# learningOrchestra/learningOrchestra

Measured on NVIDIA H100. Metric: rows/sec project+cast+histogram 100M×32 fp64→fp32; HBM GB/s vs peak @1/2/4/8 GPU, higher is better.
Workload: dtype f64->f32

## Files before the change

include/loexec.h:

```cpp
#ifndef LOEXEC_H
#define LOEXEC_H

#include <stddef.h>
#include <stdint.h>

#ifdef __cplusplus
extern "C" {
#endif

#define LO_ABI_VERSION 3

#define LO_OK                    0
#define LO_ERR_INVALID          -1
#define LO_ERR_CUDA             -2
#define LO_ERR_NOMEM            -3
#define LO_ERR_NOT_IMPLEMENTED  -4
#define LO_ERR_NO_DEVICE        -5
#define LO_ERR_ALIGNMENT        -6

#define LO_F64 1
#define LO_F32 2
#define LO_U8  3
#define LO_U32 4

// ... 43 lines not shown
                  void *base_dev, int64_t pitch_bytes, lo_table **out);
int lo_table_free(lo_ctx *ctx, lo_table *t);
int lo_table_info(const lo_table *t, int *dtype, int64_t *nrows, int32_t *ncols,
                  int64_t *pitch_bytes, void **base_dev);
int lo_table_upload_col(lo_ctx *ctx, lo_table *t, int32_t col, int64_t row0,
                        const void *host, int64_t nrows);
int lo_table_download_col(lo_ctx *ctx, const lo_table *t, int32_t col, int64_t row0,
                          void *host, int64_t nrows, void *stream);
int lo_table_fill_synthetic_dev(lo_ctx *ctx, lo_table *t, int kind, uint64_t seed,
                                int64_t row_offset, double lo, double hi, void *stream);
int lo_table_checksum(lo_ctx *ctx, const lo_table *t, int32_t col, int64_t row_offset,
                      uint64_t *out);

int lo_selftest_fastdiv(lo_ctx *ctx, float lo, float hi, int32_t nbins, int *fast_path_used,
                        uint64_t *mismatches);

int lo_project_cast_dev(lo_ctx *ctx, const lo_table *in, const int32_t *col_idx, int32_t k,
                        lo_table *out, void *stream);
int lo_project_cast_hist_dev(lo_ctx *ctx, const lo_table *in, const int32_t *col_idx, int32_t k,
                             lo_table *out, const lo_hist_spec *spec, uint64_t *counts_dev,
                             void *stream);
int lo_hist_u8_cols_dev(lo_ctx *ctx, const lo_table *in, const int32_t *col_idx, int32_t k,
                        uint64_t *counts_dev, void *stream);
int lo_minmax_cast_dev(lo_ctx *ctx, const lo_table *in, const int32_t *col_idx, int32_t k,
                       uint64_t *out_dev, void *stream);
int lo_minmax_decode(const uint64_t *raw, int32_t k, float *mins, float *maxs, uint64_t *nfinite);
int lo_counts_alloc(lo_ctx *ctx, int64_t n, uint64_t **out_dev);
int lo_counts_free(lo_ctx *ctx, uint64_t *counts_dev);
int lo_counts_zero_dev(lo_ctx *ctx, uint64_t *counts_dev, int64_t n, void *stream);
int lo_counts_download(lo_ctx *ctx, const uint64_t *counts_dev, int64_t n, uint64_t *host,
// ... 75 lines not shown
```

learningorchestra_b200/_native.py:

```python
from __future__ import annotations

import ctypes as C
from pathlib import Path

import os

LIB_PATH = Path(os.environ.get("LOEXEC_LIB") or Path(__file__).resolve().parent / "lib" / "libloexec.so")

LO_OK = 0
LO_ERR_INVALID = -1
LO_ERR_CUDA = -2
LO_ERR_NOMEM = -3
LO_ERR_NOT_IMPLEMENTED = -4
LO_ERR_NO_DEVICE = -5
LO_ERR_ALIGNMENT = -6

LO_F64, LO_F32, LO_U8, LO_U32 = 1, 2, 3, 4
LO_SYNTH_UNIFORM, LO_SYNTH_EDGES, LO_SYNTH_CONSTCOL, LO_SYNTH_MNIST_U8 = 0, 1, 2, 3
LO_MAX_BINS = 65536
LO_MERGE_AUTO, LO_MERGE_PEER, LO_MERGE_NCCL = 0, 1, 2
LO_GROUP_BCAST = 1
LO_GROUP_INDEPENDENT = 2
LO_GROUP_BLOB_BYTES = 512
LO_GROUP_MAX_DEVICES = 16
# ... 39 lines not shown
    "lo_set_tma": (C.c_int, [_P, C.c_int]),
    "lo_launch_count": (C.c_int, [_P, C.POINTER(C.c_int64)]),
    "lo_host_alloc": (C.c_int, [_P, C.c_size_t, C.POINTER(_P)]),
    "lo_host_alloc_flags": (C.c_int, [_P, C.c_size_t, C.c_int32, C.POINTER(_P)]),
    "lo_host_free": (C.c_int, [_P, _P]),
    "lo_table_alloc": (C.c_int, [_P, C.c_int, C.c_int64, C.c_int32, C.POINTER(_P)]),
    "lo_table_wrap": (C.c_int, [_P, C.c_int, C.c_int64, C.c_int32, _P, C.c_int64, C.POINTER(_P)]),
    "lo_table_free": (C.c_int, [_P, _P]),
    "lo_table_info": (C.c_int, [_P, C.POINTER(C.c_int), C.POINTER(C.c_int64), C.POINTER(C.c_int32),
                                C.POINTER(C.c_int64), C.POINTER(_P)]),
    "lo_table_upload_col": (C.c_int, [_P, _P, C.c_int32, C.c_int64, _P, C.c_int64]),
    "lo_table_download_col": (C.c_int, [_P, _P, C.c_int32, C.c_int64, _P, C.c_int64, _P]),
    "lo_table_fill_synthetic_dev": (C.c_int, [_P, _P, C.c_int, C.c_uint64, C.c_int64, C.c_double, C.c_double, _P]),
    "lo_table_checksum": (C.c_int, [_P, _P, C.c_int32, C.c_int64, C.POINTER(C.c_uint64)]),
    "lo_selftest_fastdiv": (C.c_int, [_P, C.c_float, C.c_float, C.c_int32, C.POINTER(C.c_int), C.POINTER(C.c_uint64)]),
    "lo_minmax_cast_dev": (C.c_int, [_P, _P, C.POINTER(C.c_int32), C.c_int32, _P, _P]),
    "lo_minmax_decode": (C.c_int, [_P, C.c_int32, _P, _P, _P]),
    "lo_project_cast_dev": (C.c_int, [_P, _P, C.POINTER(C.c_int32), C.c_int32, _P, _P]),
    "lo_project_cast_hist_dev": (C.c_int, [_P, _P, C.POINTER(C.c_int32), C.c_int32, _P, C.POINTER(HistSpec), _P, _P]),
    "lo_hist_u8_cols_dev": (C.c_int, [_P, _P, C.POINTER(C.c_int32), C.c_int32, _P, _P]),
    "lo_counts_alloc": (C.c_int, [_P, C.c_int64, C.POINTER(_P)]),
    "lo_counts_free": (C.c_int, [_P, _P]),
    "lo_counts_zero_dev": (C.c_int, [_P, _P, C.c_int64, _P]),
    "lo_counts_download": (C.c_int, [_P, _P, C.c_int64, _P, _P]),
    "lo_project_cast_hist_host": (C.c_int, [_P, C.POINTER(_P), C.c_int64, C.c_int32, C.POINTER(_P),
                                            C.POINTER(HistSpec), _P, C.POINTER(HostTiming)]),
    "lo_hist_u8_cols_host": (C.c_int, [_P, C.POINTER(_P), C.c_int64, C.c_int32, _P, C.POINTER(HostTiming)]),
    "lo_group_create_local": (C.c_int, [C.POINTER(_P), C.c_int32, C.c_int32, C.POINTER(_P)]),
    "lo_group_rank_begin": (C.c_int, [_P, C.c_int32, C.c_int32, C.c_int32, C.POINTER(_P), _P]),
    "lo_group_rank_connect": (C.c_int, [_P, _P]),
# ... 53 lines not shown
```

learningorchestra_b200/csrc/kernels.cuh:

```cuda
#pragma once
#include <cstdint>
#include <cuda_runtime.h>
#include "parse_number.cuh"
#include "format_number.cuh"

namespace lo {

constexpr int kThreads      = 256;
constexpr int kVec          = 4;
constexpr int kBatch        = 4;
constexpr int kBatches      = 15;
constexpr int kVecPerThread = kBatch * kBatches;
constexpr int kElemsPerThread = kVec * kVecPerThread;
constexpr int kTileRows     = kThreads * kElemsPerThread;
constexpr int kHalf         = kThreads * kVec / 2;
constexpr int kHistRows     = 64;
constexpr int kHistSmemBytes = (kHistRows * kThreads + 256) * 4;

#ifndef LO_PF_BATCH
#define LO_PF_BATCH 5
#endif
#ifndef LO_PF_NBUF
#define LO_PF_NBUF 2
#endif
// ... 133 lines not shown
    uint32_t c0 = 0, c1 = 0, c2 = 0, c3 = 0;
    if (v0) c0 = *p0;
    if (v1) c1 = *p1;
    if (v2) c2 = *p2;
    if (v3) c3 = *p3;
    c0 += 1;
    c1 += 1 + (b1 == b0);
    c2 += 1 + (b2 == b0) + (b2 == b1);
    c3 += 1 + (b3 == b0) + (b3 == b1) + (b3 == b2);
    if (v0) *p0 = (uint8_t)c0;
    if (v1) *p1 = (uint8_t)c1;
    if (v2) *p2 = (uint8_t)c2;
    if (v3) *p3 = (uint8_t)c3;
}

__device__ __forceinline__ void zero_private_own(uint32_t *smem, int rows) {
    for (int w = 0; w < rows; ++w) smem[w * kThreads + (threadIdx.x & (kThreads - 1))] = 0u;
}

__device__ __forceinline__ void zero_private(uint32_t *smem, int rows) {
    uint4 *p = reinterpret_cast<uint4 *>(smem);
    const int n = rows * (kThreads / 4);
    for (int i = threadIdx.x; i < n; i += kThreads) p[i] = make_uint4(0u, 0u, 0u, 0u);
    __syncthreads();
}

__device__ __forceinline__ void fold_and_flush(uint32_t *smem, int rows, int nbins,
                                               unsigned long long *counts ) {
    static_assert(kThreads / 32 == 8 && kHistRows == 64, "fold assumes 8 warps x 8 rows");
    uint32_t *folded = smem + kHistRows * kThreads;
// ... 6 lines not shown
        uint32_t even = 0u, odd = 0u;
        if (w < rows) {
            const uint4 a = *reinterpret_cast<const uint4 *>(smem + w * kThreads + 4 * lane);
            const uint4 b = *reinterpret_cast<const uint4 *>(smem + w * kThreads + 128 + 4 * lane);
            const uint32_t x[8] = {a.x, a.y, a.z, a.w, b.x, b.y, b.z, b.w};
#pragma unroll
            for (int q = 0; q < 8; ++q) {
                even += x[q] & 0x00FF00FFu;
                odd  += __byte_perm(x[q], 0u, 0x4341u);
            }
        }
        r[2 * i] = even;
        r[2 * i + 1] = odd;
    }
#pragma unroll
    for (int half = 8, bit = 16; half >= 1; half >>= 1, bit >>= 1) {
        const bool upper = (lane & bit) != 0;
#pragma unroll
        for (int i = 0; i < half; ++i) {
            const uint32_t send = upper ? r[i] : r[i + half];
            const uint32_t keep = upper ? r[i + half] : r[i];
            r[i] = keep + __shfl_xor_sync(0xffffffffu, send, bit);
        }
    }
    const uint32_t total = r[0] + __shfl_xor_sync(0xffffffffu, r[0], 1);
    if ((lane & 1) == 0) {
        const int idx = (lane >> 1) & 15;
        const int w = warp + 8 * (idx >> 1), parity = idx & 1;
        if (w < rows) {
            folded[4 * w + parity]     = total & 0xFFFFu;
            folded[4 * w + 2 + parity] = total >> 16;
        }
    }
    __syncthreads();
    if ((int)threadIdx.x < nbins) {
        uint32_t c = folded[threadIdx.x];
        if (c) asm volatile("red.relaxed.gpu.global.add.u64 [%0], %1;" :: "l"(counts + threadIdx.x), "l"((unsigned long long)c) : "memory");
// ... 116 lines not shown
        *sflag = (last && G.is_root) ? 2u : 0u;
        if (*sflag == 2u) {
            epilogue_turn_wait(G);
            if (!wait_flag_ge(G.arrived, G.arrive_target, G.timeout_ns, G.timed_out)) *sflag = 3u;
        }
    }
    __syncthreads();
    if (*sflag == 2u) group_root_epilogue(G, k * nb, threadIdx.x, blockDim.x, true);
    else if (*sflag == 3u && (int)threadIdx.x < G.npeers) red_release_sys_add(G.peer_clean[threadIdx.x], 1ull);
    if (*sflag >= 2u) {
        __syncthreads();
        if (threadIdx.x == 0) epilogue_turn_done(G);
    }
}

template <int OUT, bool HIST, bool ALIGNED, bool FASTDIV>
__global__ void __launch_bounds__(kThreads, LO_MIN_CTAS)
k_project_cast_hist(const char *__restrict__ in_base, long long in_pitch,
                    char *__restrict__ out_base, long long out_pitch,
                    long long nrows, unsigned tiles_per_col, unsigned long long *__restrict__ counts,
                    const __grid_constant__ ColsF64 P, const __grid_constant__ GroupStep G) {
    extern __shared__ uint32_t smem[];
    if (G.overlap) asm volatile("griddepcontrol.launch_dependents;" ::: "memory");
    const unsigned j    = blockIdx.x / tiles_per_col;
    const unsigned tile = blockIdx.x - j * tiles_per_col;
    const long long r0  = (long long)tile * kTileRows;
    const long long n   = min((long long)kTileRows, nrows - r0);

    const double *in = reinterpret_cast<const double *>(in_base + (long long)P.col[j] * in_pitch) + r0;
    float  *out32 = nullptr;
    double *out64 = nullptr;
    if (OUT == 1) out32 = reinterpret_cast<float *>(out_base + (long long)j * out_pitch) + r0;
    if (OUT == 2) out64 = reinterpret_cast<double *>(out_base + (long long)j * out_pitch) + r0;

    BinParams B = {0.f, 0.f, 1.f, 1.f, 0};
    int rows = 0;
    uint8_t *priv = reinterpret_cast<uint8_t *>(smem) + 4 * threadIdx.x;
    if (HIST) {
        B.lo = P.lo[j]; B.hi = P.hi[j]; B.w = P.w[j];
        B.r = __frcp_rn(B.w);
        B.last = P.nbins - 1;
        rows = (P.nbins + 3) >> 2;
    }

    if (ALIGNED && n == kTileRows) {
        double v[kPfBuf][kPfBatch][4];
        const double *src = in + 2 * (long long)threadIdx.x;
#pragma unroll
        for (int pb = 0; pb < kPfBuf - 1; ++pb)
#pragma unroll
            for (int u = 0; u < kPfBatch; ++u)
                ldg_split4_stream(src + (long long)(pb * kPfBatch + u) * kThreads * kVec, kHalf, v[pb][u]);
        if (HIST) zero_private(smem, rows);
#pragma unroll 1
        for (int b0 = 0; b0 < kPfBatches; b0 += kPfBuf) {
#pragma unroll
            for (int s = 0; s < kPfBuf; ++s) {
                const int b  = b0 + s;
                const int nb = b + kPfBuf - 1;
                if (nb < kPfBatches) {
#pragma unroll
                    for (int u = 0; u < kPfBatch; ++u)
                        ldg_split4_stream(src + (long long)(nb * kPfBatch + u) * kThreads * kVec, kHalf,
                                          v[(s + kPfBuf - 1) % kPfBuf][u]);
                }
#pragma unroll
                for (int u = 0; u < kPfBatch; ++u) {
                    const long long e = (long long)(b * kPfBatch + u) * kThreads * kVec + 2 * threadIdx.x;
                    float f0 = cast_f64_f32(v[s][u][0]), f1 = cast_f64_f32(v[s][u][1]);
                    float f2 = cast_f64_f32(v[s][u][2]), f3 = cast_f64_f32(v[s][u][3]);
                    if (OUT == 1) stg_split4_stream(out32 + e, kHalf, f0, f1, f2, f3);
                    if (OUT == 2) stg_split4_stream(out64 + e, kHalf, v[s][u]);
                    if (HIST)
                        bump4(priv, bin_index_f32<FASTDIV>(f0, B), bin_index_f32<FASTDIV>(f1, B),
                              bin_index_f32<FASTDIV>(f2, B), bin_index_f32<FASTDIV>(f3, B));
                }
            }
        }
    } else if (ALIGNED) {
        if (HIST) zero_private(smem, rows);
#pragma unroll 1
        for (int b = 0; b < kBatches; ++b) {
            const long long e0 = (long long)b * kBatch * kThreads * kVec + 2 * threadIdx.x;
            if (e0 >= n) break;
            double v[kBatch][4];
            if (e0 + (long long)(kBatch - 1) * kThreads * kVec + kHalf + 2 <= n) {
#pragma unroll
                for (int u = 0; u < kBatch; ++u) ldg_split4_stream(in + e0 + (long long)u * kThreads * kVec, kHalf, v[u]);
#pragma unroll
                for (int u = 0; u < kBatch; ++u) {
                    const long long e = e0 + (long long)u * kThreads * kVec;
                    float f0 = cast_f64_f32(v[u][0]), f1 = cast_f64_f32(v[u][1]);
                    float f2 = cast_f64_f32(v[u][2]), f3 = cast_f64_f32(v[u][3]);
                    if (OUT == 1) stg_split4_stream(out32 + e, kHalf, f0, f1, f2, f3);
                    if (OUT == 2) stg_split4_stream(out64 + e, kHalf, v[u]);
                    if (HIST)
                        bump4(priv, bin_index_f32<FASTDIV>(f0, B), bin_index_f32<FASTDIV>(f1, B),
                              bin_index_f32<FASTDIV>(f2, B), bin_index_f32<FASTDIV>(f3, B));
                }
            } else {
#pragma unroll 1
                for (int u = 0; u < kBatch; ++u) {
                    const long long e = e0 + (long long)u * kThreads * kVec;
#pragma unroll 1
                    for (int q = 0; q < kVec; ++q) {
                        const long long eq = e + (q & 1) + (q >> 1) * kHalf;
                        if (eq < n) {
                            double x = ldg64_stream(in + eq);
                            float  f = cast_f64_f32(x);
                            if (OUT == 1) out32[eq] = f;
                            if (OUT == 2) out64[eq] = x;
                            if (HIST) bin_f32<FASTDIV>(priv, f, B);
                        }
                    }
                }
            }
        }
    } else {
        if (HIST) zero_private(smem, rows);
#pragma unroll 1
        for (int i = 0; i < kElemsPerThread; ++i) {
            const long long e = (long long)i * kThreads + threadIdx.x;
            if (e >= n) break;
            double x = ldg64_stream(in + e);
            float  f = cast_f64_f32(x);
            if (OUT == 1) out32[e] = f;
            if (OUT == 2) out64[e] = x;
            if (HIST) bin_f32<FASTDIV>(priv, f, B);
        }
    }

    if (HIST) {
        if (G.mode == 0) {
            fold_and_flush(smem, rows, P.nbins, counts + (long long)j * P.nbins);
        } else {
            group_wait_generation(G);
            fold_and_flush(smem, rows, P.nbins, G.local + (long long)j * P.nbins);
            group_finish_column(G, j, P.nbins, P.k, tiles_per_col, smem);
        }
    }
}

constexpr int kWBThreads   = 512;
// ... 657 lines not shown
}

__global__ void k_selftest_fastdiv(float lo, float hi, float w, int nbins, unsigned long long *mismatches) {
    BinParams B = {lo, hi, w, __frcp_rn(w), nbins - 1};
    unsigned long long bad = 0;
    for (unsigned long long i = blockIdx.x * (unsigned long long)blockDim.x + threadIdx.x; i < (1ull << 32);
         i += (unsigned long long)gridDim.x * blockDim.x) {
        const float f = __uint_as_float((unsigned)i);
        bad += bin_index_f32<true>(f, B) != bin_index_f32<false>(f, B);
    }
#pragma unroll
    for (int s = 16; s > 0; s >>= 1) bad += __shfl_xor_sync(0xffffffffu, bad, s);
    if ((threadIdx.x & 31) == 0 && bad) atomicAdd(mismatches, bad);
}

template <typename T>
__global__ void k_checksum(const T *col, long long nrows, long long row_offset, unsigned long long *out) {
    unsigned long long acc = 0;
    for (long long r = blockIdx.x * (long long)blockDim.x + threadIdx.x; r < nrows;
         r += (long long)gridDim.x * blockDim.x) {
        unsigned long long bits;
        if (sizeof(T) == 8)      bits = (unsigned long long)reinterpret_cast<const unsigned long long *>(col)[r];
        else if (sizeof(T) == 4) bits = (unsigned long long)reinterpret_cast<const unsigned int *>(col)[r];
        else                     bits = (unsigned long long)reinterpret_cast<const unsigned char *>(col)[r];
        acc += bits * (2ull * (unsigned long long)(row_offset + r) + 1ull);
    }
#pragma unroll
    for (int s = 16; s > 0; s >>= 1) acc += __shfl_xor_sync(0xffffffffu, acc, s);
    if ((threadIdx.x & 31) == 0 && acc) atomicAdd(out, acc);
}
// ... 3 lines not shown
```

learningorchestra_b200/csrc/loexec.cu:

```cuda
#include "loexec.h"
#include "kernels.cuh"

#include <cub/device/device_scan.cuh>

#include <atomic>
#include <condition_variable>
#include <cctype>
#include <chrono>
#include <cmath>
#include <cstdarg>
#include <cstdio>
#include <cstdlib>
#include <cstring>
#include <mutex>
#include <new>
#include <string>
#include <utility>
#include <vector>

namespace {

thread_local std::string g_err;

int fail(int code, const char *fmt, ...) {
    char buf[512];
    va_list ap;
    va_start(ap, fmt);
    vsnprintf(buf, sizeof buf, fmt, ap);
// ... 41 lines not shown
    int       device;
};

constexpr int kSlots = 3;
constexpr int kMaxStageSets = 4;

struct StageSet {
    cudaStream_t compute = nullptr, h2d = nullptr, d2h = nullptr;
    char        *in[kSlots]  = {nullptr, nullptr, nullptr};
    char        *out[kSlots] = {nullptr, nullptr, nullptr};
    size_t       in_bytes = 0, out_bytes = 0;
    unsigned long long *counts = nullptr;
    size_t       counts_n = 0;
    cudaEvent_t  ev_h2d[kSlots] = {}, ev_k[kSlots] = {}, ev_d2h[kSlots] = {};
};

struct lo_ctx {
    int          device;
    int          sm_count;
    size_t       hbm_bytes;
    cudaStream_t stream;
    std::atomic<int64_t> launches{0};
    std::atomic<bool> use_tma{false};
    std::mutex   pool_mu;
    std::condition_variable pool_cv;
    std::vector<StageSet *> free_sets;
    int          nsets = 0;
};

namespace {

cudaStream_t pick(lo_ctx *ctx, void *stream) { return stream ? (cudaStream_t)stream : ctx->stream; }

int check_ctx(const lo_ctx *ctx) {
    if (!ctx) return fail(LO_ERR_INVALID, "ctx is NULL");
    cudaError_t e = cudaSetDevice(ctx->device);
    if (e != cudaSuccess) return fail(LO_ERR_CUDA, "cudaSetDevice(%d): %s", ctx->device, cudaGetErrorString(e));
    return LO_OK;
}

bool aligned32(const lo_table *t) {
    return ((uintptr_t)t->base % 32 == 0) && (t->pitch % 32 == 0);
// ... 14 lines not shown
    if (spec->flags != 0) return fail(LO_ERR_INVALID, "unknown lo_hist_spec.flags 0x%x", spec->flags);
    if (!spec->lo || !spec->hi) return fail(LO_ERR_INVALID, "lo_hist_spec.lo / .hi is NULL");
    for (int j = 0; j < k; ++j) {
        const float lo = spec->lo[j], hi = spec->hi[j];
        volatile float span = hi - lo;
        volatile float w    = span / (float)spec->nbins;
        if (!(std::isfinite(lo) && std::isfinite(hi)) || !(hi > lo) || !std::isfinite(w) || !(w > 0.0f))
            return fail(LO_ERR_INVALID, "histogram range of column %d is not usable: lo=%g hi=%g nbins=%d",
                        j, (double)lo, (double)hi, spec->nbins);
        w_out[j] = w;
    }
    return LO_OK;
}

template <typename K>
int allow_smem(K kernel) {
    LO_CUDA(cudaFuncSetAttribute(kernel, cudaFuncAttributeMaxDynamicSharedMemorySize, lo::kHistSmemBytes));
    return LO_OK;
}

template <int OUT>
int allow_smem_hist() {
    LO_TRY(allow_smem(lo::k_project_cast_hist<OUT, true, true, true>));
    LO_TRY(allow_smem(lo::k_project_cast_hist<OUT, true, true, false>));
    LO_TRY(allow_smem(lo::k_project_cast_hist<OUT, true, false, true>));
    LO_TRY(allow_smem(lo::k_project_cast_hist<OUT, true, false, false>));
    return LO_OK;
}

bool fastdiv_ok(float w) {
    uint32_t bits;
    memcpy(&bits, &w, 4);
    if ((bits & 0x007FFFFFu) == 0x007FFFFFu) return false;
    return w >= 0x1p-100f && w <= 0x1p100f;
}

template <typename K>
int allow_smem_tma(K kernel) {
    LO_CUDA(cudaFuncSetAttribute(kernel, cudaFuncAttributeMaxDynamicSharedMemorySize, lo::kTmaSmemBytes));
    return LO_OK;
}

int configure_kernels() {
    LO_TRY(allow_smem_tma(lo::k_project_cast_hist_tma<0, true, true>));
    LO_TRY(allow_smem_tma(lo::k_project_cast_hist_tma<1, true, true>));
    LO_TRY(allow_smem_tma(lo::k_project_cast_hist_tma<2, true, true>));
    LO_TRY(allow_smem_tma(lo::k_project_cast_hist_tma<1, false, false>));
    LO_TRY(allow_smem_tma(lo::k_project_cast_hist_tma<2, false, false>));
    LO_TRY(allow_smem_hist<0>());
// ... 19 lines not shown
    cfg.gridDim = dim3(grid);
    cfg.blockDim = dim3(block);
    cfg.dynamicSmemBytes = smem;
    cfg.stream = s;
    cudaLaunchAttribute attr[1];
    attr[0].id = cudaLaunchAttributeProgrammaticStreamSerialization;
    attr[0].val.programmaticStreamSerializationAllowed = 1;
    cfg.attrs = attr;
    cfg.numAttrs = overlap ? 1 : 0;
    return cudaLaunchKernelEx(&cfg, kernel, std::forward<Args>(args)...);
}

template <int OUT, bool HIST>
int launch_f64(lo_ctx *ctx, const lo_table *in, const lo_table *out, int32_t out_col0,
               const lo::ColsF64 &P, unsigned long long *counts, bool aligned, const lo::GroupStep &G, cudaStream_t s) {
    const size_t smem = HIST ? lo::kHistSmemBytes : 0;
    char *out_base = out ? out->base + (int64_t)out_col0 * out->pitch : nullptr;
    const long long out_pitch = out ? out->pitch : 0;
    bool fast = HIST;
    for (int j = 0; HIST && j < P.k; ++j) fast = fast && fastdiv_ok(P.w[j]);
    if (ctx->use_tma.load(std::memory_order_relaxed) && aligned && fast == HIST && in->nrows >= lo::kTileRows && G.mode == 0) {
        const unsigned full_tiles = (unsigned)(in->nrows / lo::kTileRows);
        const unsigned long long tblocks = (unsigned long long)full_tiles * (unsigned)P.k;
        if (tblocks > 0x7fffffffull) return fail(LO_ERR_INVALID, "table too large for one launch (%llu tiles)", tblocks);
        lo::k_project_cast_hist_tma<OUT, HIST, HIST><<<(unsigned)tblocks, lo::kThreads + 32, lo::kTmaSmemBytes, s>>>(
            in->base, in->pitch, out_base, out_pitch, in->nrows, full_tiles, counts, P);
        LO_CUDA(cudaGetLastError());
        ctx->launches.fetch_add(1, std::memory_order_relaxed);
        const int64_t done = (int64_t)full_tiles * lo::kTileRows;
        if (done == in->nrows) return LO_OK;
        const char *ib = in->base + done * 8;
        char *ob = out ? out->base + done * (int64_t)dtype_size(out->dtype) + (int64_t)out_col0 * out->pitch : nullptr;
        if (fast) lo::k_project_cast_hist<OUT, HIST, true, true><<<(unsigned)P.k, lo::kThreads, smem, s>>>(
                      ib, in->pitch, ob, out_pitch, in->nrows - done, 1u, counts, P, kNoGroup);
        else      lo::k_project_cast_hist<OUT, HIST, true, false><<<(unsigned)P.k, lo::kThreads, smem, s>>>(
                      ib, in->pitch, ob, out_pitch, in->nrows - done, 1u, counts, P, kNoGroup);
        LO_CUDA(cudaGetLastError());
        ctx->launches.fetch_add(1, std::memory_order_relaxed);
        return LO_OK;
    }
    const unsigned tiles_per_col = (unsigned)((in->nrows + lo::kTileRows - 1) / lo::kTileRows);
    const unsigned long long blocks = (unsigned long long)tiles_per_col * (unsigned)P.k;
    if (blocks > 0x7fffffffull) return fail(LO_ERR_INVALID, "table too large for one launch (%llu tiles)", blocks);
    const char *ib = in->base;
    const long long ip = in->pitch, nr = in->nrows;
#define LO_LAUNCH(AL, FD)                                                                                        \
    LO_CUDA(launch_kernel(lo::k_project_cast_hist<OUT, HIST, AL, FD>, (unsigned)blocks, lo::kThreads, smem, s,    \
                          G.overlap != 0, ib, ip, out_base, out_pitch, nr, tiles_per_col, counts, P, G))
    if (aligned) { if (fast) LO_LAUNCH(true, true); else LO_LAUNCH(true, false); }
    else         { if (fast) LO_LAUNCH(false, true); else LO_LAUNCH(false, false); }
#undef LO_LAUNCH
    LO_CUDA(cudaGetLastError());
    ctx->launches.fetch_add(1, std::memory_order_relaxed);
    return LO_OK;
}

template <int OUT>
int launch_f64_bins(lo_ctx *ctx, const lo_table *in, const lo_table *out, int32_t out_col0,
                    const lo::ColsF64 &P, unsigned long long *counts, bool aligned, const lo::GroupStep &G, cudaStream_t s) {
    char *out_base = out ? out->base + (int64_t)out_col0 * out->pitch : nullptr;
    const long long out_pitch = out ? out->pitch : 0;
    bool fast = true;
    for (int j = 0; j < P.k; ++j) fast = fast && fastdiv_ok(P.w[j]);
    int slots_log2 = -1;
    if (P.nbins <= lo::kWBSmemWords) {
        slots_log2 = 0;
        while (slots_log2 < 5 && (P.nbins << (slots_log2 + 1)) <= lo::kWBSmemWords) ++slots_log2;
    } else if (P.nbins <= lo::kWBSmemWordsMax) {
// ... 244 lines not shown
                    prop.major, prop.minor);
    int reserved = 0;
    LO_CUDA(cudaDeviceGetAttribute(&reserved, cudaDevAttrReservedSharedMemoryPerBlock, device));
    if (reserved != LO_SMEM_WINDOW_BASE)
        return fail(LO_ERR_NO_DEVICE, "device %d reserves %d bytes of shared memory per block, the kernels assume %d",
                    device, reserved, LO_SMEM_WINDOW_BASE);
    LO_CUDA(cudaSetDevice(device));
    lo_ctx *ctx = new (std::nothrow) lo_ctx;
    if (!ctx) return fail(LO_ERR_NOMEM, "out of host memory");
    ctx->device    = device;
    ctx->sm_count  = prop.multiProcessorCount;
    ctx->hbm_bytes = prop.totalGlobalMem;
    ctx->stream = nullptr;
    auto setup = [&]() -> int {
        LO_CUDA(cudaStreamCreateWithFlags(&ctx->stream, cudaStreamNonBlocking));
        cudaMemPool_t pool = nullptr;
        LO_CUDA(cudaDeviceGetDefaultMemPool(&pool, device));
        uint64_t keep = 8ull << 30;
        if (const char *e = getenv("LOEXEC_POOL_KEEP_MB")) keep = (uint64_t)std::max<long long>(0, atoll(e)) << 20;
        LO_CUDA(cudaMemPoolSetAttribute(pool, cudaMemPoolAttrReleaseThreshold, &keep));
        return configure_kernels();
    };
    if (const char *e = getenv("LOEXEC_TMA")) ctx->use_tma.store(e[0] == '1');
    const int rc = setup();
    if (rc != LO_OK) {
        const std::string msg = g_err;
        lo_shutdown(ctx);
        g_err = msg;
        return rc;
    }
    *out = ctx;
    return LO_OK;
}

int lo_shutdown(lo_ctx *ctx) {
    if (!ctx) return LO_OK;
    cudaSetDevice(ctx->device);
    cudaDeviceSynchronize();
    for (StageSet *st : ctx->free_sets) stage_set_destroy(st);
    ctx->free_sets.clear();
    if (ctx->stream) cudaStreamDestroy(ctx->stream);
    delete ctx;
    return LO_OK;
}

int lo_ctx_device(const lo_ctx *ctx, int *device, int *sm_count, size_t *hbm_bytes) {
    if (!ctx) return fail(LO_ERR_INVALID, "ctx is NULL");
    if (device) *device = ctx->device;
    if (sm_count) *sm_count = ctx->sm_count;
    if (hbm_bytes) *hbm_bytes = ctx->hbm_bytes;
    return LO_OK;
}

int lo_sync(lo_ctx *ctx, void *stream) {
    LO_TRY(check_ctx(ctx));
// ... 198 lines not shown
    if (fast_path_used) *fast_path_used = fastdiv_ok(w) ? 1 : 0;
    unsigned long long *d = nullptr;
    LO_CUDA(cudaMalloc((void **)&d, 8));
    cudaError_t e = cudaMemsetAsync(d, 0, 8, ctx->stream);
    if (e == cudaSuccess) {
        lo::k_selftest_fastdiv<<<ctx->sm_count * 16, 256, 0, ctx->stream>>>(lo_v, hi_v, w, nbins, d);
        e = cudaGetLastError();
        ctx->launches.fetch_add(1, std::memory_order_relaxed);
    }
    unsigned long long h = 0;
    if (e == cudaSuccess) e = cudaMemcpyAsync(&h, d, 8, cudaMemcpyDeviceToHost, ctx->stream);
    if (e == cudaSuccess) e = cudaStreamSynchronize(ctx->stream);
    cudaFree(d);
    if (e != cudaSuccess) return fail(LO_ERR_CUDA, "selftest: %s", cudaGetErrorString(e));
    *mismatches = h;
    return LO_OK;
}

int lo_minmax_cast_dev(lo_ctx *ctx, const lo_table *in, const int32_t *col_idx, int32_t k, uint64_t *out_dev, void *stream) {
    LO_TRY(check_ctx(ctx));
    if (!in || in->dtype != LO_F64) return fail(LO_ERR_INVALID, "input table must be LO_F64");
    LO_TRY(check_cols(in, col_idx, k));
    if (!out_dev) return fail(LO_ERR_INVALID, "out_dev is NULL");
    cudaStream_t s = pick(ctx, stream);
    LO_CUDA(cudaMemsetAsync(out_dev, 0, (size_t)k * 24, s));
    if (in->nrows == 0) return LO_OK;
    for (int j = 0; j < k; ++j) {
        dim3 grid((unsigned)std::min<int64_t>((in->nrows + 2047) / 2048, ctx->sm_count * 4), 1);
        lo::k_minmax_cast<<<grid, 256, 0, s>>>(in->base + (int64_t)col_idx[j] * in->pitch, in->pitch, in->nrows,
                                               (unsigned long long *)out_dev + 3 * j);
// ... 538 lines not shown
```

learningorchestra_b200/engine.py:

```python
from __future__ import annotations

import ctypes as C
from typing import Iterable, Sequence

import numpy as np

from . import _native as N

_DTYPES = {"f64": N.LO_F64, "f32": N.LO_F32, "u8": N.LO_U8}
_NP = {N.LO_F64: np.float64, N.LO_F32: np.float32, N.LO_U8: np.uint8}


def _stream_ptr(stream) -> C.c_void_p:
    if stream is None:
        return C.c_void_p(0)
    if hasattr(stream, "cuda_stream"):
        return C.c_void_p(int(stream.cuda_stream))
    return C.c_void_p(int(stream))


def _i32(col_idx: Iterable[int]):
    if isinstance(col_idx, C.Array):
        return col_idx, len(col_idx)
    idx = [int(c) for c in col_idx]
# ... 172 lines not shown
    def wrap_counts(self, k: int, nbins: int, ptr: int, keepalive=None) -> DeviceCounts:
        return DeviceCounts(self, k, nbins, ptr=ptr, keepalive=keepalive)

    def pinned_empty(self, shape, dtype, write_combined: bool = False) -> np.ndarray:
        dtype = np.dtype(dtype)
        nbytes = int(np.prod(shape)) * dtype.itemsize
        p = C.c_void_p()
        N.check(self._lib.lo_host_alloc_flags(self._ctx, max(nbytes, 1), 1 if write_combined else 0, C.byref(p)))
        self._pinned[p.value] = p
        buf = (C.c_char * max(nbytes, 1)).from_address(p.value)
        return np.frombuffer(buf, dtype=dtype, count=int(np.prod(shape))).reshape(shape)

    def selftest_fastdiv(self, lo: float, hi: float, nbins: int) -> tuple[bool, int]:
        used, bad = C.c_int(), C.c_uint64()
        N.check(self._lib.lo_selftest_fastdiv(self._ctx, float(lo), float(hi), int(nbins), C.byref(used), C.byref(bad)))
        return bool(used.value), int(bad.value)

    def _spec(self, k: int, nbins: int, lo, hi, flags: int = 0):
        lo_a = (C.c_float * k)(*[float(v) for v in np.broadcast_to(np.asarray(lo, dtype=np.float32), (k,))])
        hi_a = (C.c_float * k)(*[float(v) for v in np.broadcast_to(np.asarray(hi, dtype=np.float32), (k,))])
        spec = N.HistSpec(int(nbins), int(flags), C.cast(lo_a, C.POINTER(C.c_float)), C.cast(hi_a, C.POINTER(C.c_float)))
        return spec, (lo_a, hi_a)

    def project_cast(self, table: DeviceTable, col_idx, out: DeviceTable | None = None, out_dtype: str = "f32",
                     stream=None) -> DeviceTable:
        idx, k = _i32(col_idx)
        if out is None:
            out = self.table(out_dtype, table.nrows, k)
        N.check(self._lib.lo_project_cast_dev(self._ctx, table._h, idx, k, out._h, _stream_ptr(stream)))
        return out
# ... 190 lines not shown
```

Measured before the change: 7.280 billion.

## Replace per-element bin division with precomputed edge-table lookup in shared memory

Computes exact IEEE bin edges on the host, once per (lo, hi, nbins) spec, and caches up to eight device edge tables with LRU retirement tracked by events. The histogram kernel loads a 513-slot table into shared memory, maps each value to a slot with a scaled FMA and a float-bits trick, then picks the counter offset with one compare against the stored edge. This replaces the division or fast-reciprocal bin computation while keeping results bit-identical to the IEEE divide. The change also tightens the address arithmetic in the aligned loop and reshapes the shuffle-reduce loop. In exchange it adds shared-memory footprint, a host mutex held around every launch, and host-side edge computation on a cache miss.

Result: faster. 7.578 billion, median of 6 (+4.1%).

```diff
diff --git a/include/loexec.h b/include/loexec.h
--- a/include/loexec.h
+++ b/include/loexec.h
@@ -81,6 +81,12 @@
 
 int lo_selftest_fastdiv(lo_ctx *ctx, float lo, float hi, int32_t nbins, int *fast_path_used,
                         uint64_t *mismatches);
+
+int lo_hist_edges(float lo, float hi, int32_t nbins, float *edges);
+
+int lo_selftest_edges(lo_ctx *ctx, float lo, float hi, int32_t nbins, int *edges_used, uint64_t *mismatches);
+
+int lo_edge_tables_info(lo_ctx *ctx, int32_t *tables, uint64_t *bytes, int64_t *divide_launches);
 
 int lo_project_cast_dev(lo_ctx *ctx, const lo_table *in, const int32_t *col_idx, int32_t k,
                         lo_table *out, void *stream);
diff --git a/learningorchestra_b200/_native.py b/learningorchestra_b200/_native.py
--- a/learningorchestra_b200/_native.py
+++ b/learningorchestra_b200/_native.py
@@ -77,6 +77,9 @@
     "lo_table_fill_synthetic_dev": (C.c_int, [_P, _P, C.c_int, C.c_uint64, C.c_int64, C.c_double, C.c_double, _P]),
     "lo_table_checksum": (C.c_int, [_P, _P, C.c_int32, C.c_int64, C.POINTER(C.c_uint64)]),
     "lo_selftest_fastdiv": (C.c_int, [_P, C.c_float, C.c_float, C.c_int32, C.POINTER(C.c_int), C.POINTER(C.c_uint64)]),
+    "lo_hist_edges": (C.c_int, [C.c_float, C.c_float, C.c_int32, _P]),
+    "lo_selftest_edges": (C.c_int, [_P, C.c_float, C.c_float, C.c_int32, C.POINTER(C.c_int), C.POINTER(C.c_uint64)]),
+    "lo_edge_tables_info": (C.c_int, [_P, C.POINTER(C.c_int32), C.POINTER(C.c_uint64), C.POINTER(C.c_int64)]),
     "lo_minmax_cast_dev": (C.c_int, [_P, _P, C.POINTER(C.c_int32), C.c_int32, _P, _P]),
     "lo_minmax_decode": (C.c_int, [_P, C.c_int32, _P, _P, _P]),
     "lo_project_cast_dev": (C.c_int, [_P, _P, C.POINTER(C.c_int32), C.c_int32, _P, _P]),
diff --git a/learningorchestra_b200/csrc/kernels.cuh b/learningorchestra_b200/csrc/kernels.cuh
--- a/learningorchestra_b200/csrc/kernels.cuh
+++ b/learningorchestra_b200/csrc/kernels.cuh
@@ -171,6 +171,44 @@
     if (v3) *p3 = (uint8_t)c3;
 }
 
+constexpr int      kEdgeSlots     = 513;
+constexpr uint32_t kTrashOffset   = kHistRows * kThreads * 4;
+constexpr int      kEdgeSmemBytes = kHistSmemBytes + kEdgeSlots * 16;
+
+__device__ __forceinline__ void load_edge_table(uint4 *tab, const float *__restrict__ E, int nbins) {
+    for (int i = threadIdx.x; i < kEdgeSlots; i += blockDim.x) {
+        const float e = i <= nbins ? E[i] : __int_as_float(0x7f800000);
+        const uint32_t off0  = i < nbins ? bin_byte_offset((uint32_t)i) : kTrashOffset;
+        const uint32_t offm1 = (i >= 1 && i <= nbins) ? bin_byte_offset((uint32_t)(i - 1)) : kTrashOffset;
+        tab[i] = make_uint4(__float_as_uint(e), off0, offm1, 0u);
+    }
+}
+
+struct EdgeParams {
+    float    lo, rs;
+    uint32_t tab_bits;
+};
+
+__device__ __forceinline__ EdgeParams edge_params(float lo, float w, const uint4 *tab) {
+    const uint32_t base = __shfl_sync(0xffffffffu, (uint32_t)__cvta_generic_to_shared(tab) - 16u * 0x46800000u, 0);
+    return {lo, __frcp_rn(w) * 0x1p-9f, base};
+}
+
+__device__ __forceinline__ uint32_t edge_counter_offset(float f, const EdgeParams &E) {
+    const float t = __saturatef(__fmaf_rn(__fsub_rn(f, E.lo), E.rs, 0x1p-10f));
+    const uint32_t bits = __float_as_uint(__fadd_rz(t, 0x1p14f));
+    uint32_t e, off0, offm1, pad;
+    asm volatile("ld.shared.v4.u32 {%0,%1,%2,%3}, [%4];"
+                 : "=r"(e), "=r"(off0), "=r"(offm1), "=r"(pad) : "r"(E.tab_bits + 16u * bits));
+    asm volatile("" :: "r"(pad));
+    return f >= __uint_as_float(e) ? off0 : offm1;
+}
+
+__device__ __forceinline__ void bump_edge(uint8_t *priv, float f, const EdgeParams &E) {
+    uint8_t *p = priv + edge_counter_offset(f, E);
+    *p = (uint8_t)(*p + 1);
+}
+
 __device__ __forceinline__ void zero_private_own(uint32_t *smem, int rows) {
     for (int w = 0; w < rows; ++w) smem[w * kThreads + (threadIdx.x & (kThreads - 1))] = 0u;
 }
@@ -207,13 +245,16 @@
         r[2 * i + 1] = odd;
     }
 #pragma unroll
-    for (int half = 8, bit = 16; half >= 1; half >>= 1, bit >>= 1) {
+    for (int s = 0; s < 4; ++s) {
+        const int half = 8 >> s, bit = 16 >> s;
         const bool upper = (lane & bit) != 0;
 #pragma unroll
-        for (int i = 0; i < half; ++i) {
-            const uint32_t send = upper ? r[i] : r[i + half];
-            const uint32_t keep = upper ? r[i + half] : r[i];
-            r[i] = keep + __shfl_xor_sync(0xffffffffu, send, bit);
+        for (int i = 0; i < 8; ++i) {
+            if (i < half) {
+                const uint32_t send = upper ? r[i] : r[i + half];
+                const uint32_t keep = upper ? r[i + half] : r[i];
+                r[i] = keep + __shfl_xor_sync(0xffffffffu, send, bit);
+            }
         }
     }
     const uint32_t total = r[0] + __shfl_xor_sync(0xffffffffu, r[0], 1);
@@ -360,12 +401,12 @@
     }
 }
 
-template <int OUT, bool HIST, bool ALIGNED, bool FASTDIV>
+template <int OUT, bool HIST, bool ALIGNED, bool EDGES>
 __global__ void __launch_bounds__(kThreads, LO_MIN_CTAS)
 k_project_cast_hist(const char *__restrict__ in_base, long long in_pitch,
                     char *__restrict__ out_base, long long out_pitch,
                     long long nrows, unsigned tiles_per_col, unsigned long long *__restrict__ counts,
-                    const __grid_constant__ ColsF64 P, const __grid_constant__ GroupStep G) {
+                    const float *__restrict__ edges, const __grid_constant__ ColsF64 P, const __grid_constant__ GroupStep G) {
     extern __shared__ uint32_t smem[];
     if (G.overlap) asm volatile("griddepcontrol.launch_dependents;" ::: "memory");
     const unsigned j    = blockIdx.x / tiles_per_col;
@@ -388,6 +429,12 @@
         B.last = P.nbins - 1;
         rows = (P.nbins + 3) >> 2;
     }
+    EdgeParams E = {0.f, 0.f, 0u};
+    if (HIST && EDGES) {
+        uint4 *tab = reinterpret_cast<uint4 *>(reinterpret_cast<char *>(smem) + kHistSmemBytes);
+        load_edge_table(tab, edges + (long long)j * (P.nbins + 1), P.nbins);
+        E = edge_params(B.lo, B.w, tab);
+    }
 
     if (ALIGNED && n == kTileRows) {
         double v[kPfBuf][kPfBatch][4];
@@ -398,8 +445,12 @@
             for (int u = 0; u < kPfBatch; ++u)
                 ldg_split4_stream(src + (long long)(pb * kPfBatch + u) * kThreads * kVec, kHalf, v[pb][u]);
         if (HIST) zero_private(smem, rows);
+        const long long t2 = 2 * (long long)threadIdx.x;
 #pragma unroll 1
         for (int b0 = 0; b0 < kPfBatches; b0 += kPfBuf) {
+            const double *rsrc = src + (long long)b0 * (kPfBatch * kThreads * kVec);
+            float  *rout32 = (OUT == 1) ? out32 + t2 + (long long)b0 * (kPfBatch * kThreads * kVec) : nullptr;
+            double *rout64 = (OUT == 2) ? out64 + t2 + (long long)b0 * (kPfBatch * kThreads * kVec) : nullptr;
 #pragma unroll
             for (int s = 0; s < kPfBuf; ++s) {
                 const int b  = b0 + s;
@@ -407,19 +458,22 @@
                 if (nb < kPfBatches) {
 #pragma unroll
                     for (int u = 0; u < kPfBatch; ++u)
-                        ldg_split4_stream(src + (long long)(nb * kPfBatch + u) * kThreads * kVec, kHalf,
+                        ldg_split4_stream(rsrc + ((s + kPfBuf - 1) * kPfBatch + u) * kThreads * kVec, kHalf,
                                           v[(s + kPfBuf - 1) % kPfBuf][u]);
                 }
 #pragma unroll
                 for (int u = 0; u < kPfBatch; ++u) {
-                    const long long e = (long long)(b * kPfBatch + u) * kThreads * kVec + 2 * threadIdx.x;
+                    const int e = (s * kPfBatch + u) * kThreads * kVec;
                     float f0 = cast_f64_f32(v[s][u][0]), f1 = cast_f64_f32(v[s][u][1]);
                     float f2 = cast_f64_f32(v[s][u][2]), f3 = cast_f64_f32(v[s][u][3]);
-                    if (OUT == 1) stg_split4_stream(out32 + e, kHalf, f0, f1, f2, f3);
-                    if (OUT == 2) stg_split4_stream(out64 + e, kHalf, v[s][u]);
-                    if (HIST)
-                        bump4(priv, bin_index_f32<FASTDIV>(f0, B), bin_index_f32<FASTDIV>(f1, B),
-                              bin_index_f32<FASTDIV>(f2, B), bin_index_f32<FASTDIV>(f3, B));
+                    if (OUT == 1) stg_split4_stream(rout32 + e, kHalf, f0, f1, f2, f3);
+                    if (OUT == 2) stg_split4_stream(rout64 + e, kHalf, v[s][u]);
+                    if (HIST && EDGES) {
+                        bump_edge(priv, f0, E); bump_edge(priv, f1, E); bump_edge(priv, f2, E); bump_edge(priv, f3, E);
+                    } else if (HIST) {
+                        bump4(priv, bin_index_f32<false>(f0, B), bin_index_f32<false>(f1, B),
+                              bin_index_f32<false>(f2, B), bin_index_f32<false>(f3, B));
+                    }
                 }
             }
         }
@@ -440,9 +494,12 @@
                     float f2 = cast_f64_f32(v[u][2]), f3 = cast_f64_f32(v[u][3]);
                     if (OUT == 1) stg_split4_stream(out32 + e, kHalf, f0, f1, f2, f3);
                     if (OUT == 2) stg_split4_stream(out64 + e, kHalf, v[u]);
-                    if (HIST)
-                        bump4(priv, bin_index_f32<FASTDIV>(f0, B), bin_index_f32<FASTDIV>(f1, B),
-                              bin_index_f32<FASTDIV>(f2, B), bin_index_f32<FASTDIV>(f3, B));
+                    if (HIST && EDGES) {
+                        bump_edge(priv, f0, E); bump_edge(priv, f1, E); bump_edge(priv, f2, E); bump_edge(priv, f3, E);
+                    } else if (HIST) {
+                        bump4(priv, bin_index_f32<false>(f0, B), bin_index_f32<false>(f1, B),
+                              bin_index_f32<false>(f2, B), bin_index_f32<false>(f3, B));
+                    }
                 }
             } else {
 #pragma unroll 1
@@ -456,7 +513,8 @@
                             float  f = cast_f64_f32(x);
                             if (OUT == 1) out32[eq] = f;
                             if (OUT == 2) out64[eq] = x;
-                            if (HIST) bin_f32<FASTDIV>(priv, f, B);
+                            if (HIST && EDGES) bump_edge(priv, f, E);
+                            else if (HIST) bin_f32<false>(priv, f, B);
                         }
                     }
                 }
@@ -472,7 +530,8 @@
             float  f = cast_f64_f32(x);
             if (OUT == 1) out32[e] = f;
             if (OUT == 2) out64[e] = x;
-            if (HIST) bin_f32<FASTDIV>(priv, f, B);
+            if (HIST && EDGES) bump_edge(priv, f, E);
+            else if (HIST) bin_f32<false>(priv, f, B);
         }
     }
 
@@ -1160,6 +1219,25 @@
     if ((threadIdx.x & 31) == 0 && bad) atomicAdd(mismatches, bad);
 }
 
+__global__ void __launch_bounds__(256) k_selftest_edges(float lo, float hi, float w, int nbins, const float *edges,
+                                                        unsigned long long *mismatches) {
+    __shared__ uint4 tab[kEdgeSlots];
+    load_edge_table(tab, edges, nbins);
+    __syncthreads();
+    const EdgeParams E = edge_params(lo, w, tab);
+    const BinParams B = {lo, hi, w, __frcp_rn(w), nbins - 1};
+    unsigned long long bad = 0;
+    for (unsigned long long i = blockIdx.x * (unsigned long long)blockDim.x + threadIdx.x; i < (1ull << 32);
+         i += (unsigned long long)gridDim.x * blockDim.x) {
+        const float f = __uint_as_float((unsigned)i);
+        const int b = bin_index_f32<false>(f, B);
+        bad += edge_counter_offset(f, E) != (b >= 0 ? bin_byte_offset((uint32_t)b) : kTrashOffset);
+    }
+#pragma unroll
+    for (int s = 16; s > 0; s >>= 1) bad += __shfl_xor_sync(0xffffffffu, bad, s);
+    if ((threadIdx.x & 31) == 0 && bad) atomicAdd(mismatches, bad);
+}
+
 template <typename T>
 __global__ void k_checksum(const T *col, long long nrows, long long row_offset, unsigned long long *out) {
     unsigned long long acc = 0;
diff --git a/learningorchestra_b200/csrc/loexec.cu b/learningorchestra_b200/csrc/loexec.cu
--- a/learningorchestra_b200/csrc/loexec.cu
+++ b/learningorchestra_b200/csrc/loexec.cu
@@ -3,6 +3,7 @@
 
 #include <cub/device/device_scan.cuh>
 
+#include <algorithm>
 #include <atomic>
 #include <condition_variable>
 #include <cctype>
@@ -12,6 +13,7 @@
 #include <cstdio>
 #include <cstdlib>
 #include <cstring>
+#include <memory>
 #include <mutex>
 #include <new>
 #include <string>
@@ -83,6 +85,17 @@
     size_t       counts_n = 0;
     cudaEvent_t  ev_h2d[kSlots] = {}, ev_k[kSlots] = {}, ev_d2h[kSlots] = {};
 };
+
+struct EdgeTable {
+    int32_t            nbins = 0;
+    std::vector<float> lo, hi;
+    float             *dev = nullptr;
+    size_t             bytes = 0;
+    cudaEvent_t        ready = nullptr;
+    std::vector<cudaEvent_t> uses;
+    uint64_t           last_use = 0;
+};
+constexpr int kEdgeTables = 8;
 
 struct lo_ctx {
     int          device;
@@ -95,6 +108,11 @@
     std::condition_variable pool_cv;
     std::vector<StageSet *> free_sets;
     int          nsets = 0;
+    std::mutex   edge_mu;
+    cudaStream_t edge_stream = nullptr;
+    std::vector<std::unique_ptr<EdgeTable>> edge_tables;
+    uint64_t     edge_tick = 0;
+    std::atomic<int64_t> divide_launches{0};
 };
 
 namespace {
@@ -139,17 +157,17 @@
 }
 
 template <typename K>
-int allow_smem(K kernel) {
-    LO_CUDA(cudaFuncSetAttribute(kernel, cudaFuncAttributeMaxDynamicSharedMemorySize, lo::kHistSmemBytes));
+int allow_smem(K kernel, int bytes) {
+    LO_CUDA(cudaFuncSetAttribute(kernel, cudaFuncAttributeMaxDynamicSharedMemorySize, bytes));
     return LO_OK;
 }
 
 template <int OUT>
 int allow_smem_hist() {
-    LO_TRY(allow_smem(lo::k_project_cast_hist<OUT, true, true, true>));
-    LO_TRY(allow_smem(lo::k_project_cast_hist<OUT, true, true, false>));
-    LO_TRY(allow_smem(lo::k_project_cast_hist<OUT, true, false, true>));
-    LO_TRY(allow_smem(lo::k_project_cast_hist<OUT, true, false, false>));
+    LO_TRY(allow_smem(lo::k_project_cast_hist<OUT, true, true, true>, lo::kEdgeSmemBytes));
+    LO_TRY(allow_smem(lo::k_project_cast_hist<OUT, true, true, false>, lo::kHistSmemBytes));
+    LO_TRY(allow_smem(lo::k_project_cast_hist<OUT, true, false, true>, lo::kEdgeSmemBytes));
+    LO_TRY(allow_smem(lo::k_project_cast_hist<OUT, true, false, false>, lo::kHistSmemBytes));
     return LO_OK;
 }
 
@@ -158,6 +176,139 @@
     memcpy(&bits, &w, 4);
     if ((bits & 0x007FFFFFu) == 0x007FFFFFu) return false;
     return w >= 0x1p-100f && w <= 0x1p100f;
+}
+
+bool edges_ok(float w) { return w >= 0x1p-100f && w <= 0x1p100f; }
+
+int bin_ieee_host(float f, float lo, float w, int last) {
+    volatile float d = f - lo;
+    volatile float q = d / w;
+    const int i = (int)q;
+    return i < last ? i : last;
+}
+
+int32_t f32_key(float f) {
+    int32_t b;
+    memcpy(&b, &f, 4);
+    return b >= 0 ? b : -(b & 0x7FFFFFFF);
+}
+float key_f32(int32_t k) {
+    const uint32_t b = k >= 0 ? (uint32_t)k : (0x80000000u | (uint32_t)(-(int64_t)k));
+    float f;
+    memcpy(&f, &b, 4);
+    return f;
+}
+
+void hist_edges(float lo, float hi, float w, int32_t nbins, float *E) {
+    const int last = nbins - 1;
+    const int64_t khi = f32_key(hi);
+    const float above = std::nextafter(hi, INFINITY);
+    auto at_or_above = [&](int64_t k, int32_t i) { return bin_ieee_host(key_f32((int32_t)k), lo, w, last) >= i; };
+    E[0] = lo;
+    int64_t floor_k = f32_key(lo);
+    for (int32_t i = 1; i < nbins; ++i) {
+        if (!at_or_above(khi, i)) { E[i] = above; continue; }
+        const int64_t g = std::min(khi, std::max(floor_k, (int64_t)f32_key((float)((double)lo + (double)i * w))));
+        int64_t a, b;
+        if (at_or_above(g, i)) {
+            b = g;
+            for (int64_t step = 1;; step *= 2) {
+                a = b - step;
+                if (a < floor_k) { a = floor_k - 1; break; }
+                if (!at_or_above(a, i)) break;
+                b = a;
+            }
+        } else {
+            a = g;
+            for (int64_t step = 1;; step *= 2) {
+                b = a + step;
+                if (b >= khi) { b = khi; break; }
+                if (at_or_above(b, i)) break;
+                a = b;
+            }
+        }
+        while (b - a > 1) {
+            const int64_t m = a + (b - a) / 2;
+            if (at_or_above(m, i)) b = m; else a = m;
+        }
+        E[i] = key_f32((int32_t)b);
+        floor_k = b;
+    }
+    E[nbins] = above;
+}
+
+void edge_retire(lo_ctx *ctx, EdgeTable *t) {
+    for (cudaEvent_t e : t->uses) {
+        cudaStreamWaitEvent(ctx->edge_stream, e, 0);
+        cudaEventDestroy(e);
+    }
+    t->uses.clear();
+    if (t->ready) cudaEventDestroy(t->ready);
+    if (t->dev) cudaFreeAsync(t->dev, ctx->edge_stream);
+    t->ready = nullptr;
+    t->dev = nullptr;
+}
+
+int edge_acquire(lo_ctx *ctx, const lo::ColsF64 &P, cudaStream_t s, EdgeTable **out) {
+    *out = nullptr;
+    for (int j = 0; j < P.k; ++j)
+        if (!edges_ok(P.w[j])) return LO_OK;
+    EdgeTable *t = nullptr;
+    for (const auto &c : ctx->edge_tables)
+        if (c->nbins == P.nbins && (int)c->lo.size() == P.k && std::equal(c->lo.begin(), c->lo.end(), P.lo) &&
+            std::equal(c->hi.begin(), c->hi.end(), P.hi)) {
+            t = c.get();
+            break;
+        }
+    if (!t) {
+        if ((int)ctx->edge_tables.size() >= kEdgeTables) {
+            auto lru = std::min_element(ctx->edge_tables.begin(), ctx->edge_tables.end(),
+                                        [](const auto &x, const auto &y) { return x->last_use < y->last_use; });
+            edge_retire(ctx, lru->get());
+            ctx->edge_tables.erase(lru);
+        }
+        auto nt = std::make_unique<EdgeTable>();
+        nt->nbins = P.nbins;
+        nt->lo.assign(P.lo, P.lo + P.k);
+        nt->hi.assign(P.hi, P.hi + P.k);
+        const size_t n = (size_t)P.k * (P.nbins + 1);
+        nt->bytes = n * 4;
+        std::vector<float> h(n);
+        for (int j = 0; j < P.k; ++j) hist_edges(P.lo[j], P.hi[j], P.w[j], P.nbins, h.data() + (size_t)j * (P.nbins + 1));
+        cudaError_t e = cudaMallocAsync((void **)&nt->dev, nt->bytes, ctx->edge_stream);
+        if (e == cudaSuccess) e = cudaMemcpyAsync(nt->dev, h.data(), nt->bytes, cudaMemcpyHostToDevice, ctx->edge_stream);
+        if (e == cudaSuccess) e = cudaEventCreateWithFlags(&nt->ready, cudaEventDisableTiming);
+        if (e == cudaSuccess) e = cudaEventRecord(nt->ready, ctx->edge_stream);
+        if (e != cudaSuccess) {
+            edge_retire(ctx, nt.get());
+            return fail(e == cudaErrorMemoryAllocation ? LO_ERR_NOMEM : LO_ERR_CUDA, "edge table upload: %s",
+                        cudaGetErrorString(e));
+        }
+        t = nt.get();
+        ctx->edge_tables.push_back(std::move(nt));
+    }
+    LO_CUDA(cudaStreamWaitEvent(s, t->ready, 0));
+    t->last_use = ++ctx->edge_tick;
+    *out = t;
+    return LO_OK;
+}
+
+int edge_used(EdgeTable *t, cudaStream_t s) {
+    t->uses.erase(std::remove_if(t->uses.begin(), t->uses.end(), [](cudaEvent_t e) {
+                      if (cudaEventQuery(e) != cudaSuccess) return false;
+                      cudaEventDestroy(e);
+                      return true;
+                  }), t->uses.end());
+    (void)cudaGetLastError();
+    cudaEvent_t e = nullptr;
+    LO_CUDA(cudaEventCreateWithFlags(&e, cudaEventDisableTiming));
+    const cudaError_t r = cudaEventRecord(e, s);
+    if (r != cudaSuccess) {
+        cudaEventDestroy(e);
+        return fail(LO_ERR_CUDA, "edge table use: %s", cudaGetErrorString(r));
+    }
+    t->uses.push_back(e);
+    return LO_OK;
 }
 
 template <typename K>
@@ -207,7 +358,18 @@
 template <int OUT, bool HIST>
 int launch_f64(lo_ctx *ctx, const lo_table *in, const lo_table *out, int32_t out_col0,
                const lo::ColsF64 &P, unsigned long long *counts, bool aligned, const lo::GroupStep &G, cudaStream_t s) {
-    const size_t smem = HIST ? lo::kHistSmemBytes : 0;
+    std::unique_lock<std::mutex> edge_lock(ctx->edge_mu, std::defer_lock);
+    EdgeTable *et = nullptr;
+    if (HIST) {
+        edge_lock.lock();
+        LO_TRY(edge_acquire(ctx, P, s, &et));
+        if (!et) {
+            edge_lock.unlock();
+            ctx->divide_launches.fetch_add(1, std::memory_order_relaxed);
+        }
+    }
+    const float *edges = et ? et->dev : nullptr;
+    const size_t smem = !HIST ? 0 : edges ? lo::kEdgeSmemBytes : lo::kHistSmemBytes;
     char *out_base = out ? out->base + (int64_t)out_col0 * out->pitch : nullptr;
     const long long out_pitch = out ? out->pitch : 0;
     bool fast = HIST;
@@ -224,12 +386,13 @@
         if (done == in->nrows) return LO_OK;
         const char *ib = in->base + done * 8;
         char *ob = out ? out->base + done * (int64_t)dtype_size(out->dtype) + (int64_t)out_col0 * out->pitch : nullptr;
-        if (fast) lo::k_project_cast_hist<OUT, HIST, true, true><<<(unsigned)P.k, lo::kThreads, smem, s>>>(
-                      ib, in->pitch, ob, out_pitch, in->nrows - done, 1u, counts, P, kNoGroup);
-        else      lo::k_project_cast_hist<OUT, HIST, true, false><<<(unsigned)P.k, lo::kThreads, smem, s>>>(
-                      ib, in->pitch, ob, out_pitch, in->nrows - done, 1u, counts, P, kNoGroup);
+        if (edges) lo::k_project_cast_hist<OUT, HIST, true, true><<<(unsigned)P.k, lo::kThreads, smem, s>>>(
+                       ib, in->pitch, ob, out_pitch, in->nrows - done, 1u, counts, edges, P, kNoGroup);
+        else       lo::k_project_cast_hist<OUT, HIST, true, false><<<(unsigned)P.k, lo::kThreads, smem, s>>>(
+                       ib, in->pitch, ob, out_pitch, in->nrows - done, 1u, counts, edges, P, kNoGroup);
         LO_CUDA(cudaGetLastError());
         ctx->launches.fetch_add(1, std::memory_order_relaxed);
+        if (et) LO_TRY(edge_used(et, s));
         return LO_OK;
     }
     const unsigned tiles_per_col = (unsigned)((in->nrows + lo::kTileRows - 1) / lo::kTileRows);
@@ -237,14 +400,15 @@
     if (blocks > 0x7fffffffull) return fail(LO_ERR_INVALID, "table too large for one launch (%llu tiles)", blocks);
     const char *ib = in->base;
     const long long ip = in->pitch, nr = in->nrows;
-#define LO_LAUNCH(AL, FD)                                                                                        \
-    LO_CUDA(launch_kernel(lo::k_project_cast_hist<OUT, HIST, AL, FD>, (unsigned)blocks, lo::kThreads, smem, s,    \
-                          G.overlap != 0, ib, ip, out_base, out_pitch, nr, tiles_per_col, counts, P, G))
-    if (aligned) { if (fast) LO_LAUNCH(true, true); else LO_LAUNCH(true, false); }
-    else         { if (fast) LO_LAUNCH(false, true); else LO_LAUNCH(false, false); }
+#define LO_LAUNCH(AL, ED)                                                                                        \
+    LO_CUDA(launch_kernel(lo::k_project_cast_hist<OUT, HIST, AL, ED>, (unsigned)blocks, lo::kThreads, smem, s,    \
+                          G.overlap != 0, ib, ip, out_base, out_pitch, nr, tiles_per_col, counts, edges, P, G))
+    if (aligned) { if (edges) LO_LAUNCH(true, true); else LO_LAUNCH(true, false); }
+    else         { if (edges) LO_LAUNCH(false, true); else LO_LAUNCH(false, false); }
 #undef LO_LAUNCH
     LO_CUDA(cudaGetLastError());
     ctx->launches.fetch_add(1, std::memory_order_relaxed);
+    if (et) LO_TRY(edge_used(et, s));
     return LO_OK;
 }
 
@@ -519,6 +683,7 @@
     ctx->stream = nullptr;
     auto setup = [&]() -> int {
         LO_CUDA(cudaStreamCreateWithFlags(&ctx->stream, cudaStreamNonBlocking));
+        LO_CUDA(cudaStreamCreateWithFlags(&ctx->edge_stream, cudaStreamNonBlocking));
         cudaMemPool_t pool = nullptr;
         LO_CUDA(cudaDeviceGetDefaultMemPool(&pool, device));
         uint64_t keep = 8ull << 30;
@@ -544,6 +709,12 @@
     cudaDeviceSynchronize();
     for (StageSet *st : ctx->free_sets) stage_set_destroy(st);
     ctx->free_sets.clear();
+    if (ctx->edge_stream) {
+        for (const auto &t : ctx->edge_tables) edge_retire(ctx, t.get());
+        cudaStreamSynchronize(ctx->edge_stream);
+        cudaStreamDestroy(ctx->edge_stream);
+    }
+    ctx->edge_tables.clear();
     if (ctx->stream) cudaStreamDestroy(ctx->stream);
     delete ctx;
     return LO_OK;
@@ -772,6 +943,56 @@
     cudaFree(d);
     if (e != cudaSuccess) return fail(LO_ERR_CUDA, "selftest: %s", cudaGetErrorString(e));
     *mismatches = h;
+    return LO_OK;
+}
+
+int lo_hist_edges(float lo_v, float hi_v, int32_t nbins, float *edges) {
+    if (!edges) return fail(LO_ERR_INVALID, "edges is NULL");
+    lo_hist_spec spec = {nbins, 0, &lo_v, &hi_v};
+    float w = 0.f;
+    LO_TRY(check_spec(&spec, 1, &w));
+    hist_edges(lo_v, hi_v, w, nbins, edges);
+    return LO_OK;
+}
+
+int lo_edge_tables_info(lo_ctx *ctx, int32_t *tables, uint64_t *bytes, int64_t *divide_launches) {
+    if (!ctx) return fail(LO_ERR_INVALID, "ctx is NULL");
+    std::lock_guard<std::mutex> g(ctx->edge_mu);
+    uint64_t b = 0;
+    for (const auto &t : ctx->edge_tables) b += t->bytes;
+    if (tables) *tables = (int32_t)ctx->edge_tables.size();
+    if (bytes) *bytes = b;
+    if (divide_launches) *divide_launches = ctx->divide_launches.load(std::memory_order_relaxed);
+    return LO_OK;
+}
+
+int lo_selftest_edges(lo_ctx *ctx, float lo_v, float hi_v, int32_t nbins, int *edges_used, uint64_t *mismatches) {
+    LO_TRY(check_ctx(ctx));
+    if (!mismatches) return fail(LO_ERR_INVALID, "mismatches is NULL");
+    if (nbins > LO_TILE_BINS) return fail(LO_ERR_INVALID, "nbins = %d: the edge-table kernels take <= %d", nbins, LO_TILE_BINS);
+    lo_hist_spec spec = {nbins, 0, &lo_v, &hi_v};
+    float w = 0.f;
+    LO_TRY(check_spec(&spec, 1, &w));
+    if (edges_used) *edges_used = edges_ok(w) ? 1 : 0;
+    std::vector<float> h((size_t)nbins + 1);
+    hist_edges(lo_v, hi_v, w, nbins, h.data());
+    unsigned long long *d = nullptr;
+    float *E = nullptr;
+    LO_CUDA(cudaMalloc((void **)&d, 8 + h.size() * 4));
+    E = reinterpret_cast<float *>(d + 1);
+    cudaError_t e = cudaMemcpyAsync(E, h.data(), h.size() * 4, cudaMemcpyHostToDevice, ctx->stream);
+    if (e == cudaSuccess) e = cudaMemsetAsync(d, 0, 8, ctx->stream);
+    if (e == cudaSuccess) {
+        lo::k_selftest_edges<<<ctx->sm_count * 16, 256, 0, ctx->stream>>>(lo_v, hi_v, w, nbins, E, d);
+        e = cudaGetLastError();
+        ctx->launches.fetch_add(1, std::memory_order_relaxed);
+    }
+    unsigned long long bad = 0;
+    if (e == cudaSuccess) e = cudaMemcpyAsync(&bad, d, 8, cudaMemcpyDeviceToHost, ctx->stream);
+    if (e == cudaSuccess) e = cudaStreamSynchronize(ctx->stream);
+    cudaFree(d);
+    if (e != cudaSuccess) return fail(LO_ERR_CUDA, "selftest: %s", cudaGetErrorString(e));
+    *mismatches = bad;
     return LO_OK;
 }
 
diff --git a/learningorchestra_b200/engine.py b/learningorchestra_b200/engine.py
--- a/learningorchestra_b200/engine.py
+++ b/learningorchestra_b200/engine.py
@@ -210,6 +210,16 @@
     def selftest_fastdiv(self, lo: float, hi: float, nbins: int) -> tuple[bool, int]:
         used, bad = C.c_int(), C.c_uint64()
         N.check(self._lib.lo_selftest_fastdiv(self._ctx, float(lo), float(hi), int(nbins), C.byref(used), C.byref(bad)))
+        return bool(used.value), int(bad.value)
+
+    def edge_tables_info(self) -> tuple[int, int, int]:
+        n, b, d = C.c_int32(), C.c_uint64(), C.c_int64()
+        N.check(self._lib.lo_edge_tables_info(self._ctx, C.byref(n), C.byref(b), C.byref(d)))
+        return int(n.value), int(b.value), int(d.value)
+
+    def selftest_edges(self, lo: float, hi: float, nbins: int) -> tuple[bool, int]:
+        used, bad = C.c_int(), C.c_uint64()
+        N.check(self._lib.lo_selftest_edges(self._ctx, float(lo), float(hi), int(nbins), C.byref(used), C.byref(bad)))
         return bool(used.value), int(bad.value)
 
     def _spec(self, k: int, nbins: int, lo, hi, flags: int = 0):
```
